# wenyuqing/panacea

Hardware: AMD Instinct MI355X
Metric: denoising steps/s (6-view x 8-frame 256x512) (higher is better)
Workload: dtype f16; 1 GPU; BASELINE config 3: Panacea+ stage-2 UNet+ControlNet, CFG 2 x 8 frames, 6 views, latent 32x384, hint 256x3072, Euler/LegacyDDPM 50-step schedule; precision=precise: split(stream,gn_stt,ff_out,stem,gn_head,gnt)+e4m3-lo, parallelism=single, graph=False, streams=2, hoisted_step_invariants=False, fused_step_tail=True

## Files before the change

panacea_amd/csrc/gemm_dispatch.h:

```cpp
#pragma once
#include "gemm_kernel.h"

namespace pnc_gemm {

template <unsigned EPI, bool WS>
static int launch_ln(const PncGemmParams& p, hipStream_t st, TileChoice tc, const void* wlo16) {
    if (tc.tile == T_256x320) return launch<PNC_A_PLAIN, 256, 320, 4, 2, 2, false, EPI, WS>(p, st, 1, wlo16);
    return launch<PNC_A_PLAIN, 128, 128, 2, 2, 2, true, EPI, WS>(p, st, 1, wlo16);
}

template <bool WS>
int dispatch_plain(const PncGemmParams& p, unsigned epi, hipStream_t st, bool* ln_fused, const void* wlo16) {
    constexpr int AM = PNC_A_PLAIN;
    const TileChoice tc = choose_tile(p);
    if (epi & E_LN) {
        if (ln_whole_rows(p, tc)) *ln_fused = true;
        else epi &= ~E_LN;
    }
    if (tc.tile == T_128x32 && epi != E_O16 && epi != E_O32) epi = E_GENERIC;
    if constexpr (!WS) {
        if (tc.tile == T_256x320 && tc.ksplit == 1 && plain_persist_ok(p, epi)) {
            switch (epi) {
                case E_O16: return launch_plain_persist<E_O16>(p, st);
                case E_O16 | E_VT: return launch_plain_persist<E_O16 | E_VT>(p, st);
// ... 15 lines not shown
    switch (epi) {
        case E_O16: return launch_tile<AM, E_O16, WS>(p, st, tc, wlo16);
        case E_O16 | E_VT: return launch_tile<AM, E_O16 | E_VT, WS>(p, st, tc, wlo16);
        case E_O32: return launch_tile<AM, E_O32, WS>(p, st, tc, wlo16);
        case E_O32 | E_O16: return launch_tile<AM, E_O32 | E_O16, WS>(p, st, tc, wlo16);
        case E_R1 | E_O32: return launch_tile<AM, E_R1 | E_O32, WS>(p, st, tc, wlo16);
        case E_R1 | E_O32 | E_O16: return launch_tile<AM, E_R1 | E_O32 | E_O16, WS>(p, st, tc, wlo16);
        case E_R1 | E_O16: return launch_tile<AM, E_R1 | E_O16, WS>(p, st, tc, wlo16);
        case E_RB | E_O32: return launch_tile<AM, E_RB | E_O32, WS>(p, st, tc, wlo16);
        case E_O32 | E_LN: return launch_ln<E_O32 | E_LN, WS>(p, st, tc, wlo16);
        case E_RB | E_O32 | E_LN: return launch_ln<E_RB | E_O32 | E_LN, WS>(p, st, tc, wlo16);
        case E_R1 | E_O32 | E_LN: return launch_ln<E_R1 | E_O32 | E_LN, WS>(p, st, tc, wlo16);
        case E_GEGLU | E_O16:
            if (tc.tile == T_256x256 && geglu_persist_ok(p)) return launch_geglu_persist<256, 256, 4, 2, WS>(p, st, wlo16);
            return launch_tile<AM, E_GEGLU | E_O16, WS>(p, st, tc, wlo16);
        case E_O16 | E_GELU:
            if constexpr (!WS) {
                if (tc.tile == T_256x256) return launch<AM, 256, 256, 4, 2, 2, true, E_O16 | E_GELU>(p, st);
                return launch<AM, 128, 128, 2, 2, 2, true, E_O16 | E_GELU>(p, st);
            }
            break;
        default: break;
    }
    return launch_tile<AM, E_GENERIC, WS>(p, st, tc, wlo16);
}

template <bool WS>
int dispatch_conv3x3(const PncGemmParams& p, unsigned epi, hipStream_t st, const void* wlo16) {
    constexpr int AM = PNC_A_CONV3X3;
    if (const int geometry = conv3x3_tile_geometry(p, epi)) return dispatch_conv3x3_tiles<WS>(p, epi, geometry, st, wlo16);
    const TileChoice tc = choose_tile(p);
    if (tc.tile == T_128x32 && epi != E_O16 && epi != E_O32) epi = E_GENERIC;
    switch (epi) {
        case E_O16: return launch_tile<AM, E_O16, WS>(p, st, tc, wlo16);
        case E_O32: return launch_tile<AM, E_O32, WS>(p, st, tc, wlo16);
        case E_O32 | E_O16: return launch_tile<AM, E_O32 | E_O16, WS>(p, st, tc, wlo16);
        case E_R1 | E_O32: return launch_tile<AM, E_R1 | E_O32, WS>(p, st, tc, wlo16);
        case E_R1 | E_O32 | E_O16: return launch_tile<AM, E_R1 | E_O32 | E_O16, WS>(p, st, tc, wlo16);
        default: return launch_tile<AM, E_GENERIC, WS>(p, st, tc, wlo16);
    }
}

static inline bool gn_stats_in_epilogue(const PncGemmParams& p, const TileChoice& tc) {
    const int cpg = p.N / 32;
    return tc.tile == T_256x320 && (p.N % 320) == 0 && (160 % cpg) == 0 && (cpg % 2) == 0 && (p.Npix % 64) == 0 && (p.M % 64) == 0 &&
           pnc_get_option(PNC_OPT_GEMM_GN_STATS) != 0;
}

template <bool WS>
int dispatch_conv1d(const PncGemmParams& p, unsigned epi, hipStream_t st, const void* wlo16) {
    constexpr int AM = PNC_A_CONV1D_T;
    TileChoice tc = choose_tile(p);
    if (tc.tile == T_128x32) epi = E_GENERIC;
    if (p.gn_part) {
        if (gn_stats_in_epilogue(p, tc)) {
            switch (epi) {
                case E_R1 | E_RB | E_O32: return launch<AM, 256, 320, 4, 2, 2, false, E_R1 | E_RB | E_O32 | E_GS, WS>(p, st, 1, wlo16);
                case E_R1 | E_R2 | E_O32: return launch<AM, 256, 320, 4, 2, 2, false, E_R1 | E_R2 | E_O32 | E_GS, WS>(p, st, 1, wlo16);
                case E_R1 | E_R2 | E_O32 | E_O16: return launch<AM, 256, 320, 4, 2, 2, false, E_R1 | E_R2 | E_O32 | E_O16 | E_GS, WS>(p, st, 1, wlo16);
                default: break;
            }
        }
        PncGemmParams q = p;
        q.gn_part = nullptr;
        const int rc = dispatch_conv1d<WS>(q, epi, st, wlo16);
        if (rc != PNC_OK) return rc;
        return pnc_groupnorm_stats(p.out32, p.ldc32, p.M / p.Npix, p.Npix, p.N, 64, p.gn_part, st);
    }
    switch (epi) {
        case E_R1 | E_RB | E_O32: return launch_tile<AM, E_R1 | E_RB | E_O32, WS>(p, st, tc, wlo16);
        case E_R1 | E_R2 | E_O32: return launch_tile<AM, E_R1 | E_R2 | E_O32, WS>(p, st, tc, wlo16);
        case E_R1 | E_R2 | E_O32 | E_O16: return launch_tile<AM, E_R1 | E_R2 | E_O32 | E_O16, WS>(p, st, tc, wlo16);
        default: return launch_tile<AM, E_GENERIC, WS>(p, st, tc, wlo16);
    }
}

}
```

panacea_amd/csrc/gemm_glds_body.inc:

```
    PncGemmParams p = pin;
    constexpr int NW = WGM * WGN;
    constexpr int MI = BM / WGM / 32, NI = BN / WGN / 32;
    constexpr int RPI = NW * 8;
    constexpr int A_IT = BM / RPI, B_IT = BN / RPI;
    constexpr int LOADS = A_IT + B_IT;
    constexpr int A_BYTES = BM * 128, B_BYTES = BN * 128, STAGE = A_BYTES + B_BYTES;
    static_assert(BM % RPI == 0 && BN % RPI == 0, "tile rows must be a multiple of the DMA row group");
    constexpr int ENI = NI < 2 ? NI : 2;
    constexpr int EPITCH = ENI * 32 + 4;
    constexpr bool GEGLU = (EPI & E_GEGLU) != 0;
    extern __shared__ __attribute__((aligned(16))) char smem[];

    const half_t* __restrict__ A = reinterpret_cast<const half_t*>(p.A);
    const half_t* __restrict__ A_lo = reinterpret_cast<const half_t*>(p.A_lo);
    const half_t* __restrict__ Wt = reinterpret_cast<const half_t*>(p.W);

    const int tiles_n = (p.N + BN - 1) / BN;
    const int tiles_m = (p.M + BM - 1) / BM;
    const int ntile_mn = tiles_m * tiles_n;
    int kslice = 0, tile, part = 0;
    if (ksplit > 1) {
        const int blk = xcd_remap(blockIdx.x, ntile_mn * ksplit);
        kslice = blk / ntile_mn; tile = blk - kslice * ntile_mn;
    } else if ((int)blockIdx.x < nfull) {
// ... 388 lines not shown
            for (int kt = 0; kt < nt_w; ++kt) {
                const bool ahead = (kt + 2) < ntot;
                if (ahead) issue_tile(kt + 2, st == 0 ? 2 : st - 1);
                if (wave_on) {
                    compute(st);
                    if (kt + 1 == nt_w) scale_lo();
                }
                if (ahead) asm volatile("s_waitcnt vmcnt(%0)" ::"n"(LOADS) : "memory");
                else asm volatile("s_waitcnt vmcnt(0)" ::: "memory");
                asm volatile("s_waitcnt lgkmcnt(0)" ::: "memory");
                __builtin_amdgcn_s_barrier();
                st = (st == 2) ? 0 : st + 1;
            }
        }
        for (int kt = nt_w; kt < n8; ++kt) {
            const bool ahead = (kt + 2) < ntot;
            if (ahead) issue_tile(kt + 2, st == 0 ? 2 : st - 1);
            if (wave_on) compute8(st, kt - nt_w);
            if (ahead) asm volatile("s_waitcnt vmcnt(%0)" ::"n"(LOADS) : "memory");
            else asm volatile("s_waitcnt vmcnt(0)" ::: "memory");
            asm volatile("s_waitcnt lgkmcnt(0)" ::: "memory");
            __builtin_amdgcn_s_barrier();
            st = (st == 2) ? 0 : st + 1;
        }
        for (int kt = n8; kt < ntot; ++kt) {
            const bool ahead = (kt + 2) < ntot;
            if (ahead) issue_tile(kt + 2, st == 0 ? 2 : st - 1);
            if (wave_on) {
                compute(st);
                if (!WS && !lo8 && kt + 1 == nt_lo) scale_lo();
            }
            if (ahead) asm volatile("s_waitcnt vmcnt(%0)" ::"n"(LOADS) : "memory");
            else asm volatile("s_waitcnt vmcnt(0)" ::: "memory");
            asm volatile("s_waitcnt lgkmcnt(0)" ::: "memory");
            __builtin_amdgcn_s_barrier();
            st = (st == 2) ? 0 : st + 1;
        }
    }

    if (!wave_on) return;
    const int mw = m0 + wm * (MI * 32), nw = n0 + wn * (NI * 32);
    if constexpr ((EPI & E_GENERIC) != 0) {
        epi_generic<MI, NI>(p, acc, lane, mw, nw);
    } else {
        if constexpr ((EPI & E_VT) != 0) {
            if (n0 >= p.n_split) { epi_vt<MI, NI>(p, acc, lane, mw, nw); return; }
        }
        if constexpr (EPI == (E_R1 | E_O32) || EPI == E_O32) {
            if (direct_epi && p.act == PNC_ACT_NONE && m0 + BM <= p.M && n0 + BN <= p.N && !split_rows && ksplit == 1) {
                epi_direct_o32<MI, NI, (EPI & E_R1) != 0>(p, acc, lane, RowLinear{mw}, nw);
                return;
            }
        }
        float* ep = reinterpret_cast<float*>(smem) + wave * (32 * EPITCH);
        __syncthreads();
        if constexpr (GEGLU) {
            epi_geglu<MI, NI>(p, acc, ep, lane, mw, nw, reinterpret_cast<const float*>(smem + RING_BYTES));
        } else {
            if constexpr ((EPI & E_LN) != 0) {
                static_assert(WGN == 2, "the fused LayerNorm pairs the two waves of a row");
                float2* lnb = reinterpret_cast<float2*>(reinterpret_cast<float*>(smem) + NW * (32 * EPITCH));
                epi_fast<MI, NI, EPI>(p, acc, ep, lane, RowLinear{mw}, nw, p.N, lnb + wave * 64, lnb + (wave ^ 1) * 64);
            } else {
                float* gs_tab = reinterpret_cast<float*>(smem) + NW * (32 * EPITCH) + wave * (NI * 16);
                epi_fast<MI, NI, (EPI & ~E_VT)>(p, acc, ep, lane, RowLinear{mw}, nw, (EPI & E_VT) ? p.n_split : p.N, nullptr, nullptr,
                                                (EPI & E_GS) ? gs_tab : nullptr);
            }
        }
    }
```

panacea_amd/csrc/gemm_kernel.h:

```cpp
#pragma once
#include "common.h"
#include <atomic>
#include <utility>

namespace pnc_gemm {

constexpr int BK = 64;
constexpr int BK8 = 128;
typedef int i32x4 __attribute__((ext_vector_type(4)));
typedef int i32x8 __attribute__((ext_vector_type(8)));
constexpr int E8M0_LO_INV = 127 - 11;

enum : unsigned {
    E_R1 = 1,
    E_R2 = 2,
    E_RB = 4,
    E_O32 = 8,
    E_O16 = 16,
    E_VT = 32,
    E_GEGLU = 64,
    E_GENERIC = 128,
    E_GELU = 256,
    E_LN = 512,
    E_GS = 1024
// ... 94 lines not shown
        int tap, ci;
        if ((p.Cin & 63) == 0) {
            const int cc = kc / 192, r = kc - cc * 192;
            tap = r >> 6; ci = (cc << 6) + (r & 63);
        } else {
            tap = kc / p.Cin; ci = kc - tap * p.Cin;
        }
        const int tt = s.y + tap - 1;
        return (!p.t_halo && (tt < 0 || tt >= p.T)) ? PNC_BUF_OOB : (unsigned)(s.rel + (tap - 1) * p.Npix * p.Cin + ci) * ESZ;
    }
}

__device__ __forceinline__ f32x4 ld4(const float* p) { return *reinterpret_cast<const f32x4*>(p); }

__device__ __forceinline__ float gelu_erf_f(float v) { return 0.5f * v * (1.0f + erff(v * 0.70710678118654752440f)); }
__device__ __attribute__((noinline)) static float gelu_erf_call(float v) { return gelu_erf_f(v); }

__device__ __forceinline__ void store_h8(half_t* out16, void* out16_lo, int64_t off, const float (&v)[8], int lo_fmt = PNC_LO_F16) {
    half8v o;
#pragma unroll
    for (int e = 0; e < 8; ++e) o[e] = (half_t)v[e];
    *reinterpret_cast<half8v*>(out16 + off) = o;
    if (out16_lo) {
        float r[8];
#pragma unroll
        for (int e = 0; e < 8; ++e) r[e] = (v[e] - (float)o[e]) * LO_SCALE;
        if (lo_fmt == PNC_LO_E4M3) {
            uint2 w;
            w.x = pack4_e4m3(r[0], r[1], r[2], r[3]);
            w.y = pack4_e4m3(r[4], r[5], r[6], r[7]);
            *reinterpret_cast<uint2*>(reinterpret_cast<char*>(out16_lo) + off) = w;
        } else {
            half8v l;
#pragma unroll
            for (int e = 0; e < 8; ++e) l[e] = (half_t)r[e];
            *reinterpret_cast<half8v*>(reinterpret_cast<half_t*>(out16_lo) + off) = l;
        }
    }
}

struct RowLinear {
    int mw;
    __device__ __forceinline__ int operator()(int lr) const { return mw + lr; }
};
template <int TWS>
struct RowHalo {
    int base, W, lr0;
    __device__ __forceinline__ int operator()(int lr) const {
        const int R = lr0 + lr;
        return base + (R >> TWS) * W + (R & ((1 << TWS) - 1));
    }
};

template <int MI, int NI, unsigned EPI, class RM = RowLinear>
__device__ __forceinline__ void epi_fast(const PncGemmParams& p, f32x16 (&acc)[MI][NI], float* ep, int lane,
                                         RM rmap, int nw, int ncols, float2* ln_mine = nullptr,
                                         const float2* ln_partner = nullptr, float* gs_tab = nullptr) {
    constexpr bool R1 = (EPI & E_R1) != 0, R2 = (EPI & E_R2) != 0, RB = (EPI & E_RB) != 0;
    constexpr bool O32 = (EPI & E_O32) != 0, O16 = (EPI & E_O16) != 0, LN = (EPI & E_LN) != 0;
    constexpr bool GS = (EPI & E_GS) != 0;
    static_assert(!GS || (O32 && !LN), "statistics of the fp32 output; not next to the fused LayerNorm");
    const int cpg = GS ? (p.N >> 5) : 1;
    if constexpr (GS) {
        gs_tab[lane] = 0.0f;
        if (lane + 64 < NI * 16) gs_tab[lane + 64] = 0.0f;
    }
    static_assert(!LN || O32, "the fused LayerNorm normalises the fp32 output it has just written");
    constexpr bool HAS_X = R1 || RB, HAS_Y = R1 && (R2 || RB);
    static_assert(!(R2 && !R1), "a single residual is passed as res1");
    static_assert(!(R1 && R2 && RB), "three added streams run the generic epilogue");
    constexpr int ENI = NI < 2 ? NI : 2;
    constexpr int EPITCH = ENI * 32 + 4;
    constexpr int NJ = (NI + ENI - 1) / ENI, NS = NJ * MI;
    constexpr int NPMAX = ENI == 2 ? 4 : 2;
    half_t* out16 = reinterpret_cast<half_t*>(p.out16);
    void* out16_lo = p.out16_lo;
    constexpr bool GELU = (EPI & E_GELU) != 0;
    const bool silu = (!HAS_X) && (p.act == PNC_ACT_SILU);
    const f32x4 z4 = {0.0f, 0.0f, 0.0f, 0.0f};
    f32x4 x0[NPMAX], x1[NPMAX], y0[NPMAX], y1[NPMAX];
    if constexpr (LN) {
        if (lane < MI * 32) ln_mine[lane] = make_float2(0.0f, 0.0f);
    }

    auto load_xy = [&](auto s_, auto ps_) {
        constexpr int s = decltype(s_)::value, ps = decltype(ps_)::value;
        constexpr int jc = (s / MI) * ENI, i = s % MI, cw = (NI - jc) < ENI ? (NI - jc) : ENI;
        constexpr int CPL = cw * 4, RPP = 64 / CPL;
        const int cl = lane % CPL, rl = lane / CPL;
        const int ncol = nw + jc * 32 + cl * 8;
        const int m = rmap(i * 32 + ps * RPP + rl);
        const bool on = (m < p.M) && (ncol < ncols);
        if constexpr (HAS_X) {
            x0[ps] = z4; x1[ps] = z4;
            if (on) {
                const float* xp = R1 ? p.res1 + (int64_t)m * p.ldr1 + ncol
                                     : p.rowbias + (int64_t)((m / p.rb_rows) % p.rb_mod) * p.N + ncol;
                x0[ps] = ld4(xp); x1[ps] = ld4(xp + 4);
            }
        }
        if constexpr (HAS_Y) {
            y0[ps] = z4; y1[ps] = z4;
            if (on) {
                const float* yp = R2 ? p.res2 + (int64_t)m * p.ldr2 + ncol
                                     : p.rowbias + (int64_t)((m / p.rb_rows) % p.rb_mod) * p.N + ncol;
                y0[ps] = ld4(yp); y1[ps] = ld4(yp + 4);
// ... 77 lines not shown
                float* dst = ep + (ps * RPP + rl) * EPITCH + cl * 8;
                *reinterpret_cast<f32x4*>(dst) = f32x4{v[0], v[1], v[2], v[3]};
                *reinterpret_cast<f32x4*>(dst + 4) = f32x4{v[4], v[5], v[6], v[7]};
            }
            if constexpr (GS) {
                if (on) {
#pragma unroll
                    for (int k = 0; k < 4; ++k) {
                        gP[k] += v[2 * k] + v[2 * k + 1];
                        gQ[k] += fmaf(v[2 * k], v[2 * k], v[2 * k + 1] * v[2 * k + 1]);
                    }
                }
            }
            if (!on) return;
            if constexpr (O32) {
                float* op = p.out32 + (int64_t)m * p.ldc32 + ncol;
                const f32x4 o0 = {v[0], v[1], v[2], v[3]}, o1 = {v[4], v[5], v[6], v[7]};
                *reinterpret_cast<f32x4*>(op) = o0;
                *reinterpret_cast<f32x4*>(op + 4) = o1;
            }
            if constexpr (O16) store_h8(out16, out16_lo, (int64_t)m * p.ldc16 + ncol, v, p.out_lo_fmt);
        });
        if constexpr (GS) {
            const int nA = min(8, (ncol / cpg + 1) * cpg - ncol);
            float sA = 0.0f, qA = 0.0f, sB = 0.0f, qB = 0.0f;
#pragma unroll
            for (int k = 0; k < 4; ++k) {
                const bool a = 2 * k < nA;
                sA += a ? gP[k] : 0.0f; qA += a ? gQ[k] : 0.0f;
                sB += a ? 0.0f : gP[k]; qB += a ? 0.0f : gQ[k];
            }
#pragma unroll
            for (int o = CPL; o < 64; o <<= 1) {
                sA += __shfl_xor(sA, o, 64); qA += __shfl_xor(qA, o, 64);
                sB += __shfl_xor(sB, o, 64); qB += __shfl_xor(qB, o, 64);
            }
            if (lane < CPL) {
                f32x4* e = reinterpret_cast<f32x4*>(gs_tab + (jc * 4 + cl) * 4);
                f32x4 t = *e;
                t[0] += sA; t[1] += qA; t[2] += sB; t[3] += qB;
                *e = t;
            }
        }
        if constexpr (LN) {
            asm volatile("s_waitcnt lgkmcnt(0)" ::: "memory");
            static_for<cw>([&](auto j_) {
                constexpr int j = decltype(j_)::value;
#pragma unroll
                for (int r = 0; r < 16; ++r)
                    acc[i][jc + j][r] = ep[mfma32_row(r, lane) * EPITCH + j * 32 + (lane & 31)];
            });
        }
    });
    if constexpr (GS) {
        asm volatile("s_waitcnt lgkmcnt(0)" ::: "memory");
        const int m_first = rmap(0);
        if (lane < (NI * 32) / cpg && m_first < p.M) {
            const int c0 = (lane * cpg) >> 3, c1 = ((lane + 1) * cpg - 1) >> 3;
            float S = 0.0f, Q = 0.0f;
            for (int c = c0; c <= c1; ++c) {
                const f32x4 t = *reinterpret_cast<const f32x4*>(gs_tab + c * 4);
                const bool first = (c * 8) / cpg == lane;
                S += first ? t[0] : t[2];
                Q += first ? t[1] : t[3];
            }
            const float n = (float)(MI * 32 * cpg);
            const float mean = S / n;
            const int f = m_first / p.Npix, chunk = (m_first - f * p.Npix) / (MI * 32), nrec = p.Npix / (MI * 32);
            float* o = p.gn_part + ((int64_t)(f * nrec + chunk) * 32 + nw / cpg + lane) * 3;
            o[0] = n; o[1] = mean; o[2] = fmaxf(Q - S * mean, 0.0f);
        }
    }
    if constexpr (LN) {
        __syncthreads();
        half_t* lnout = reinterpret_cast<half_t*>(p.ln_out16);
        const float invn = 1.0f / (float)p.N;
        static_for<NS>([&](auto s_) {
            constexpr int s = decltype(s_)::value, jc = (s / MI) * ENI, i = s % MI;
            constexpr int cw = (NI - jc) < ENI ? (NI - jc) : ENI;
            constexpr int CPL = cw * 4, RPP = 64 / CPL, NP = 32 / RPP;
            const int cl = lane % CPL, rl = lane / CPL;
            const int ncol = nw + jc * 32 + cl * 8;
            const bool col_on = ncol < ncols;
            f32x4 g0 = z4, g1 = z4, h0 = z4, h1 = z4;
            if (col_on) {
                g0 = ld4(p.ln_gamma + ncol); g1 = ld4(p.ln_gamma + ncol + 4);
                h0 = ld4(p.ln_beta + ncol); h1 = ld4(p.ln_beta + ncol + 4);
            }
            asm volatile("s_waitcnt lgkmcnt(0)" ::: "memory");
            static_for<cw>([&](auto j_) {
                constexpr int j = decltype(j_)::value;
#pragma unroll
                for (int r = 0; r < 16; ++r)
                    ep[mfma32_row(r, lane) * EPITCH + j * 32 + (lane & 31)] = acc[i][jc + j][r];
            });
            asm volatile("s_waitcnt lgkmcnt(0)" ::: "memory");
            f32x4 w0[NP], w1[NP];
#pragma unroll
            for (int ps = 0; ps < NP; ++ps) {
                const float* src = ep + (ps * RPP + rl) * EPITCH + cl * 8;
                w0[ps] = ld4(src); w1[ps] = ld4(src + 4);
            }
#pragma unroll
            for (int ps = 0; ps < NP; ++ps) {
                const int r = i * 32 + ps * RPP + rl;
                const int m = rmap(r);
                if (!(col_on && m < p.M)) continue;
                const float2 a = ln_mine[r], b = ln_partner[r];
                const float mean = (a.x + b.x) * invn;
                const float var = fmaxf(fmaf(-mean, mean, (a.y + b.y) * invn), 0.0f);
                const float rs = rsqrtf(var + p.ln_eps);
                float y[8];
#pragma unroll
                for (int e = 0; e < 4; ++e) {
                    y[e] = fmaf((w0[ps][e] - mean) * rs, g0[e], h0[e]);
                    y[e + 4] = fmaf((w1[ps][e] - mean) * rs, g1[e], h1[e]);
                }
                store_h8(lnout, nullptr, (int64_t)m * p.ldln + ncol, y);
            }
        });
    }
}

template <int MI, int NI>
__device__ __forceinline__ void epi_geglu(const PncGemmParams& p, f32x16 (&acc)[MI][NI], float* ep, int lane,
// ... 122 lines not shown
            snd.h = grp ? he : ho;
            rcv.w.x = __shfl_xor(snd.w.x, 32, 64);
            rcv.w.y = __shfl_xor(snd.w.y, 32, 64);
            half8v o8;
#pragma unroll
            for (int q = 0; q < 4; ++q) {
                o8[q] = grp ? rcv.h[q] : he[q];
                o8[4 + q] = grp ? ho[q] : rcv.h[q];
            }
            const int m8 = mw + i * 32 + 8 * (2 * rp + grp);
            if (col_on && m8 < p.M) {
                const int g = m8 / p.t_rows, t0 = m8 - g * p.t_rows;
                *reinterpret_cast<half8v*>(out16t + (int64_t)g * p.t_gstride + (int64_t)(n - p.n_split) * p.ldt + t0) = o8;
            }
        }
    });
}

template <int MI, int NI, bool R1, class RM>
__device__ __forceinline__ void epi_direct_o32(const PncGemmParams& p, f32x16 (&acc)[MI][NI], int lane, RM rmap, int nw) {
    const int col = lane & 31, h4 = 4 * (lane >> 5);
    const int m00 = rmap(0);
    const buffer_rsrc_t ro = make_rsrc(p.out32 + (int64_t)m00 * p.ldc32, 0x7FFFFF00u);
    const buffer_rsrc_t rr = make_rsrc(R1 ? p.res1 + (int64_t)m00 * p.ldr1 : p.out32, 0x7FFFFF00u);
    int vo[MI], vr[MI];
#pragma unroll
    for (int i = 0; i < MI; ++i) {
        const int dm = rmap(i * 32 + h4) - m00;
        vo[i] = (dm * p.ldc32 + nw + col) * 4;
        vr[i] = R1 ? (dm * p.ldr1 + nw + col) * 4 : 0;
    }
    unsigned x[2][16];
    auto load_res = [&](auto b_) {
        constexpr int b = decltype(b_)::value, i = b / NI, j = b % NI;
#pragma unroll
        for (int r = 0; r < 16; ++r) {
            const int so = (rmap((r & 3) + 8 * (r >> 2)) - m00) * p.ldr1 * 4;
            x[b & 1][r] = __builtin_amdgcn_raw_buffer_load_b32(rr, vr[i] + j * 128, so, 0);
        }
    };
    if constexpr (R1) load_res(std::integral_constant<int, 0>{});
    static_for<MI * NI>([&](auto b_) {
        constexpr int b = decltype(b_)::value, i = b / NI, j = b % NI;
        const float bn = p.bias ? p.bias[nw + j * 32 + col] : 0.0f;
        if constexpr (R1 && b + 1 < MI * NI) load_res(std::integral_constant<int, b + 1>{});
#pragma unroll
        for (int r = 0; r < 16; ++r) {
            float v = acc[i][j][r] + bn;
            if constexpr (R1) v += __builtin_bit_cast(float, x[b & 1][r]);
            const int so = (rmap((r & 3) + 8 * (r >> 2)) - m00) * p.ldc32 * 4;
            __builtin_amdgcn_raw_buffer_store_b32(__builtin_bit_cast(unsigned, v), ro, vo[i] + j * 128, so, 0);
        }
    });
}

template <int MI, int NI>
__device__ __forceinline__ void epi_generic(const PncGemmParams& p, f32x16 (&acc)[MI][NI], int lane, int mw, int nw) {
    half_t* out16 = reinterpret_cast<half_t*>(p.out16);
    half_t* out16_lo = reinterpret_cast<half_t*>(p.out16_lo);
    half_t* out16t = reinterpret_cast<half_t*>(p.out16t);
    const int col = lane & 31;
    static_for<MI * NI>([&](auto ij_) {
        constexpr int i = decltype(ij_)::value / NI, j = decltype(ij_)::value % NI;
        const int n = nw + j * 32 + col;
        if (n >= p.N) return;
        const float bn = p.bias ? p.bias[n] : 0.0f;
        const bool to_t = out16t && n >= p.n_split;
#pragma unroll 4
        for (int r = 0; r < 16; ++r) {
            const int m = mw + i * 32 + mfma32_row(r, lane);
            if (m >= p.M) continue;
            float v = acc[i][j][r] + bn;
            if (p.rowbias) v += p.rowbias[(int64_t)((m / p.rb_rows) % p.rb_mod) * p.N + n];
            if (p.act == PNC_ACT_SILU) v = silu_f(v);
            if (p.act == PNC_ACT_GELU) v = gelu_erf_call(v);
            if (p.res1) v += p.res1[(int64_t)m * p.ldr1 + n];
            if (p.res2) v += p.res2[(int64_t)m * p.ldr2 + n];
            if (to_t) {
                const int g = m / p.t_rows, t = m - g * p.t_rows;
                out16t[(int64_t)g * p.t_gstride + (int64_t)(n - p.n_split) * p.ldt + t] = (half_t)v;
                continue;
            }
            if (p.out32) p.out32[(int64_t)m * p.ldc32 + n] = v;
            if (out16) {
                const half_t h = (half_t)v;
                out16[(int64_t)m * p.ldc16 + n] = h;
                if (out16_lo) {
                    const float r = (v - (float)h) * LO_SCALE;
                    if (p.out_lo_fmt == PNC_LO_E4M3)
                        reinterpret_cast<unsigned char*>(p.out16_lo)[(int64_t)m * p.ldc16 + n] = (unsigned char)(pack4_e4m3(r, 0.0f, 0.0f, 0.0f) & 0xFFu);
                    else out16_lo[(int64_t)m * p.ldc16 + n] = (half_t)r;
                }
            }
        }
    });
}

template <int AMODE, int BM, int BN, int WGM, int WGN, int STAGES, bool PIPE, unsigned EPI>
__global__ __launch_bounds__(64 * WGM * WGN) void gemm_glds_kernel(const PncGemmParams pin, const int ksplit,
                                                                   const int nfull, const int tail_f,
                                                                   const float* __restrict__ phi_g, const int group_m,
                                                                   const int stagger_min_in) {
    constexpr bool WS = false;
    const void* const wlo16 = nullptr;
#include "gemm_glds_body.inc"
}
// ... 452 lines not shown
            if (nxt && !late) issue(m0, n0, kt + 1, (sp + kt + 1) & 1);
            compute((sp + kt) & 1, m0, n0, (nxt && late) ? kt + 1 : -1, (sp + kt + 1) & 1);
            __syncthreads();
        }
        const int vn = v + gridDim.x;
        int m1 = 0, n1 = 0;
        if (vn < ntile) {
            tile_origin(vn, m1, n1);
            issue(m1, n1, 0, 1);
        }
        if constexpr ((EPI & E_VT) != 0) {
            if (n0 >= p.n_split) epi_vt<MI, NI>(p, acc, lane, m0 + wm * (MI * 32), n0 + wn * (NI * 32));
            else epi_fast_alds<MI, NI, (EPI & ~E_VT)>(p, acc, ep, lane, m0 + wm * (MI * 32), n0 + wn * (NI * 32), 0u, 0u);
        } else if constexpr (EPI == E_O32 || EPI == (E_R1 | E_O32)) {
            if (!(group_m_in & 0x10000) && p.act == PNC_ACT_NONE)
                epi_direct_o32<MI, NI, (EPI & E_R1) != 0>(p, acc, lane, RowLinear{m0 + wm * (MI * 32)}, n0 + wn * (NI * 32));
            else
                epi_fast_alds<MI, NI, EPI>(p, acc, ep, lane, m0 + wm * (MI * 32), n0 + wn * (NI * 32), lnb + (unsigned)wave * 512u,
                                           lnb + (unsigned)(wave ^ 1) * 512u);
        } else {
            epi_fast_alds<MI, NI, EPI>(p, acc, ep, lane, m0 + wm * (MI * 32), n0 + wn * (NI * 32), lnb + (unsigned)wave * 512u,
                                       lnb + (unsigned)(wave ^ 1) * 512u);
        }
        if (vn >= ntile) break;
        alds_wait0();
        v = vn; m0 = m1; n0 = n1; sp = 1;
    }
}

static inline bool plain_persist_ok(const PncGemmParams& p, unsigned epi) {
    if ((pnc_get_option(PNC_OPT_GEMM_PERSIST) & 2) == 0 || p.a_mode != PNC_A_PLAIN) return false;
    if ((p.M % 256) || (p.N % 320) || (p.K % 64) || p.K < 64) return false;
    if (p.A_lo && (p.a_lo_fmt != PNC_LO_E4M3 || (p.lda % 16))) return false;
    if ((epi & E_LN) && p.N != 320) return false;
    if ((epi & E_VT) && ((p.n_split % 320) || (p.M % 8) || (p.t_rows % 8))) return false;
    return (p.M / 256) * (p.N / 320) >= 512;
}

template <unsigned EPI>
int launch_plain_persist(const PncGemmParams& p, hipStream_t st) {
    constexpr int lds = 2 * (256 + 320) * 128;
    static std::atomic<unsigned char> attr_done[64];
    const int dev = current_device();
    auto kern = gemm_persist_kernel<EPI>;
    set_dynamic_lds_once(attr_done, dev, kern, lds);
    const int tiles_n = p.N / 320, tiles_m = p.M / 256, tiles = tiles_m * tiles_n;
    const int group_m = grouped_tile_order(tiles_m, tiles_n);
    const int ncu = cu_count(dev);
    const int blocks = tiles < ncu ? tiles : ncu;
    hipLaunchKernelGGL(kern, dim3(blocks), dim3(512), lds, st, p, group_m | ((pnc_get_option(PNC_OPT_GEMM_FUSE_LN) & 2) ? 0x10000 : 0));
    return pnc_launch_status();
}

template <int AMODE, int BM, int BN, int WGM, int WGN, int STAGES, bool PIPE, unsigned EPI, bool WS = false>
int launch(const PncGemmParams& p, hipStream_t st, int ksplit = 1, const void* wlo16 = nullptr) {
    constexpr int lds = STAGES * (BM + BN) * 128;
    constexpr int threads = 64 * WGM * WGN;
    constexpr bool GEGLU = (EPI & E_GEGLU) != 0;
    static_assert(lds + (GEGLU ? PHI_BYTES : 0) <= 160 * 1024, "LDS budget of one CU (operand ring + GEGLU table)");
    static_assert(lds >= WGM * WGN * (32 * 68 * 4 + 64 * 8), "epilogue staging (+ LayerNorm row sums) must fit the operand ring");
    static std::atomic<unsigned char> attr_done[64];
    const auto kern = [] {
        if constexpr (WS) return gemm_glds_ws_kernel<AMODE, BM, BN, WGM, WGN, STAGES, PIPE, EPI>;
        else return gemm_glds_kernel<AMODE, BM, BN, WGM, WGN, STAGES, PIPE, EPI>;
    }();
    set_dynamic_lds_once(attr_done, current_device(), kern, lds + (GEGLU ? PHI_BYTES : 0));
    const int tiles =((p.M + BM - 1) / BM) * ((p.N + BN - 1) / BN);
    int nfull = tiles, tail_f = 1;
    if (ksplit == 1) tail_split<BM, WGM, lds>(tiles, nfull, tail_f);
    const int blocks = ksplit > 1 ? tiles * ksplit : nfull + (tiles - nfull) * tail_f;
    PncGemmParams q = p;
    const float* phi = nullptr;
    if constexpr (GEGLU) {
        int rc = PNC_OK;
        phi = phi_table_device(st, &rc);
        if (rc != PNC_OK) return rc;
    }
    if (ksplit > 1) {
        q.ldc32 = p.N;
        q.bias = nullptr; q.rowbias = nullptr; q.res1 = nullptr; q.res2 = nullptr;
        q.out16 = nullptr; q.out16_lo = nullptr; q.out16t = nullptr; q.n_split = p.N; q.act = PNC_ACT_NONE;
    }
    const int group_m = grouped_tile_order((p.M + BM - 1) / BM, (p.N + BN - 1) / BN);
    const int stagger = (pnc_get_option(PNC_OPT_GEMM_STAGGER) & 0xFF) | ((pnc_get_option(PNC_OPT_GEMM_FUSE_LN) & 2) ? 0 : 0x100);
    launch_kernel<WS>(kern, dim3(blocks), dim3(threads), lds + (GEGLU ? PHI_BYTES : 0), st, wlo16, q, ksplit, nfull, tail_f, phi, group_m, stagger);
    if (ksplit > 1) return launch_splitk_reduce(p, ksplit, st);
    return pnc_launch_status();
}

static inline double tile_score(long tiles, int slots, double eff) {
    if (tiles <= 0) return 0.0;
    const long q = tiles / slots, r = tiles % slots;
    const double tail = r == 0 ? 0.0 : (r * 4 <= slots ? 0.45 : (r * 2 <= slots ? 0.65 : 1.0));
    return eff * ((double)tiles / slots) / ((double)q + tail);
}

static inline int splitk_slices(const PncGemmParams& p) {
    if (p.geglu || p.out16t || (p.N % 256) || (p.N % 8)) return 1;
    if ((p.out32 && (p.ldc32 % 4)) || (p.out16 && (p.ldc16 % 8))) return 1;
    const long tiles = (long)((p.M + 255) / 256) * (p.N / 256);
    const int ktiles = (p.K + BK - 1) / BK;
    if (tiles > 96 || ktiles < 48) return 1;
    return ktiles >= 320 ? 8 : (ktiles >= 56 ? 4 : 2);
}

enum { T_128x128 = 1, T_256x128 = 2, T_256x320 = 3, T_256x256 = 4, T_128x32 = 5 };
// ... 52 lines not shown
```

panacea_amd/csrc/misc.hip:

```cpp
#include "common.h"
#include <atomic>

namespace {

constexpr int SM_MAXM = 16;

__global__ __launch_bounds__(256) void linear_smallm_kernel(const float* __restrict__ a, int lda,
                                                            const half_t* __restrict__ W,
                                                            const half_t* __restrict__ W_lo,
                                                            const float* __restrict__ bias,
                                                            float* __restrict__ out, int ldo, int M, int N,
                                                            int K, int silu_in, int silu_out) {
    const int lane = threadIdx.x & 63;
    const int n = blockIdx.x * 4 + (threadIdx.x >> 6);
    if (n >= N) return;
    float acc[SM_MAXM];
#pragma unroll
    for (int m = 0; m < SM_MAXM; ++m) acc[m] = 0.0f;
    for (int k0 = lane * 8; k0 < K; k0 += 64 * 8) {
        const half8v w = *reinterpret_cast<const half8v*>(W + (int64_t)n * K + k0);
        float wf[8];
#pragma unroll
        for (int e = 0; e < 8; ++e) wf[e] = (float)w[e];
        if (W_lo) {
// ... 329 lines not shown
    case PNC_SAMPLER_LMS:
        nv = 2 + p.n_hist;
        ok = p.out_aux && p.n_hist >= 0 && p.n_hist <= 3;
        for (int k = 0; ok && k < p.n_hist; ++k) ok = p.hist[k] != nullptr;
        break;
    default: return PNC_EINVAL;
    }
    for (int k = 0; ok && k < nv; ++k) ok = p.v[k] != nullptr;
    if (!ok) return PNC_EINVAL;
    return launch_1d(skip ? cfg_sampler_step_kernel<true> : cfg_sampler_step_kernel<false>, (int64_t)p.T * p.Npix, stream, p,
                     c_skip);
}

int cfg_euler_step_launch(const float* eps_tok, int ld, int T, int Npix, int C, int cfg, float scale, const float* x,
                          const float* c_out, const float* sigma, const float* sigma_next, float* x_next, const float* c_skip,
                          bool skip, void* stream) {
    PncSamplerStepParams p = {};
    p.struct_bytes = (int32_t)sizeof(PncSamplerStepParams);
    p.mode = PNC_SAMPLER_HEUN1;
    p.eps_tok = eps_tok, p.ld = ld, p.T = T, p.Npix = Npix, p.C = C, p.cfg = cfg, p.scale = scale;
    p.x = x, p.c_out = c_out, p.v[0] = sigma, p.v[1] = sigma_next, p.out = x_next;
    return cfg_sampler_step_launch(&p, c_skip, skip, true, stream);
}

}

extern "C" int pnc_cfg_euler_step(const float* eps_tok, int ld, int T, int Npix, int C, int cfg, float scale,
                                  const float* x, const float* c_out, const float* sigma, const float* sigma_next,
                                  float* x_next, void* stream) {
    return cfg_euler_step_launch(eps_tok, ld, T, Npix, C, cfg, scale, x, c_out, sigma, sigma_next, x_next, nullptr, false, stream);
}

extern "C" int pnc_cfg_euler_step_skip(const float* eps_tok, int ld, int T, int Npix, int C, int cfg, float scale,
                                       const float* x, const float* c_skip, const float* c_out, const float* sigma,
                                       const float* sigma_next, float* x_next, void* stream) {
    return cfg_euler_step_launch(eps_tok, ld, T, Npix, C, cfg, scale, x, c_out, sigma, sigma_next, x_next, c_skip, true, stream);
}

extern "C" int pnc_cfg_sampler_step(const PncSamplerStepParams* pp, void* stream) {
    return cfg_sampler_step_launch(pp, nullptr, false, false, stream);
}

extern "C" int pnc_cfg_sampler_step_skip(const PncSamplerStepParams* pp, const float* c_skip, void* stream) {
    return cfg_sampler_step_launch(pp, c_skip, true, false, stream);
}

extern "C" const char* pnc_version(void) { return "panacea_hip 0.4.0 gfx950"; }
#ifndef PNC_BUILD_DIGEST
#define PNC_BUILD_DIGEST "unstamped"
#endif
static const char k_build_digest[] = "pnc-build-digest:" PNC_BUILD_DIGEST;
extern "C" const char* pnc_build_digest(void) { return k_build_digest + 17; }

static std::atomic<int> g_options[PNC_OPT_COUNT] = {{1}, {0}, {0}, {1}, {1}, {0}, {1}, {3}, {8}, {1}, {4}, {12}};

int pnc_get_option(int option) { return g_options[option].load(std::memory_order_relaxed); }

extern "C" int pnc_set_option(int option, int value) {
    if (option < 0 || option >= PNC_OPT_COUNT) return PNC_EINVAL;
    return g_options[option].exchange(value, std::memory_order_relaxed);
}

extern "C" int pnc_linear_smallm_split(const float* a, int lda, const void* W, const void* W_lo, const float* bias,
                                       float* out, int ldo, int M, int N, int K, int silu_in, int silu_out,
                                       void* stream) {
    if (!a || !W || !out || M < 1 || M > SM_MAXM || N < 1 || K < 8) return PNC_EINVAL;
    if (K % 8 || lda % 4) return PNC_EINVAL;
    if (((uintptr_t)a | (uintptr_t)W | (uintptr_t)W_lo) & 15) return PNC_EALIGN;
    return launch_1d(linear_smallm_kernel, (int64_t)N * 64, stream, a, lda, f16p(W), f16p(W_lo), bias, out, ldo, M, N, K, silu_in,
                     silu_out);
}

extern "C" int pnc_linear_smallm(const float* a, int lda, const void* W, const float* bias,
                                 float* out, int ldo, int M, int N, int K, int silu_in, int silu_out,
                                 void* stream) {
    return pnc_linear_smallm_split(a, lda, W, nullptr, bias, out, ldo, M, N, K, silu_in, silu_out, stream);
}

extern "C" int pnc_linear_smallm_segments(const float* a, int lda, const void* W, const float* bias, float* out, int M,
                                          int m0, int Mtot, int N, int K, const int32_t* seg_start, int nseg, int silu_in,
                                          int silu_out, void* stream) {
    return pnc_linear_smallm_segments_split(a, lda, W, nullptr, bias, out, M, m0, Mtot, N, K, seg_start, nseg, silu_in, silu_out, stream);
}

extern "C" int pnc_linear_smallm_segments_split(const float* a, int lda, const void* W, const void* W_lo, const float* bias,
                                                float* out, int M, int m0, int Mtot, int N, int K, const int32_t* seg_start,
                                                int nseg, int silu_in, int silu_out, void* stream) {
    if (!a || !W || !out || !seg_start || M < 1 || M > SM_MAXM || m0 < 0 || m0 + M > Mtot || N < 1 || K < 8) return PNC_EINVAL;
    if (K % 8 || lda % 4 || nseg < 1 || nseg > PNC_SMALLM_MAX_SEGS) return PNC_EINVAL;
    if (((uintptr_t)a | (uintptr_t)W | (uintptr_t)W_lo) & 15) return PNC_EALIGN;
    SmallmSegs segs;
    segs.nseg = nseg;
    if (seg_start[0] != 0 || seg_start[nseg] != N) return PNC_EINVAL;
    for (int i = 0; i <= nseg; ++i) {
        if (seg_start[i] % SEG_NC || (i > 0 && seg_start[i] <= seg_start[i - 1])) return PNC_EINVAL;
        segs.start[i] = seg_start[i];
    }
    return launch_1d(linear_smallm_seg_kernel, (int64_t)(N / SEG_NC) * 64, stream, a, lda, f16p(W), f16p(W_lo), bias, out, M, m0, Mtot,
                     N, K, silu_in, silu_out, segs);
}

template <typename TS>
static int timestep_embedding(const TS* t, int F, int dim, const float* freqs, float* out, void* stream) {
    if (!t || !out || !freqs || F < 1 || dim < 2) return PNC_EINVAL;
    return launch_1d(timestep_embedding_kernel<TS>, F * (dim / 2), stream, t, F, dim, freqs, out);
}

// ... 122 lines not shown
```

Measured before the change: 6.408 steps/s.

## Add persistent conv1d temporal GEMM kernel with direct residual and GN-stats epilogue

Adds a persistent conv1d (temporal) GEMM kernel for 256x320 tiles. It prefetches the next tile's first K-stage while the current tile's epilogue runs. It also adds a direct-to-global epilogue that fuses bias, row bias or second residual and GroupNorm partial statistics using DPP lane reductions, skipping the LDS staging round-trip. The default persist option is changed from 3 to 7 to enable the path, which adds code complexity and a new reduction ordering for GN statistics.

```diff
diff --git a/panacea_amd/csrc/gemm_dispatch.h b/panacea_amd/csrc/gemm_dispatch.h
--- a/panacea_amd/csrc/gemm_dispatch.h
+++ b/panacea_amd/csrc/gemm_dispatch.h
@@ -91,6 +91,17 @@
     constexpr int AM = PNC_A_CONV1D_T;
     TileChoice tc = choose_tile(p);
     if (tc.tile == T_128x32) epi = E_GENERIC;
+    if constexpr (!WS) {
+        if (tc.tile == T_256x320 && tc.ksplit == 1 && conv1d_persist_ok(p, epi) && (!p.gn_part || gn_stats_in_epilogue(p, tc))) {
+            switch (epi | (p.gn_part ? (unsigned)E_GS : 0u)) {
+                case E_R1 | E_RB | E_O32: return launch_conv1d_persist<E_R1 | E_RB | E_O32>(p, st);
+                case E_R1 | E_R2 | E_O32: return launch_conv1d_persist<E_R1 | E_R2 | E_O32>(p, st);
+                case E_R1 | E_RB | E_O32 | E_GS: return launch_conv1d_persist<E_R1 | E_RB | E_O32 | E_GS>(p, st);
+                case E_R1 | E_R2 | E_O32 | E_GS: return launch_conv1d_persist<E_R1 | E_R2 | E_O32 | E_GS>(p, st);
+                default: break;
+            }
+        }
+    }
     if (p.gn_part) {
         if (gn_stats_in_epilogue(p, tc)) {
             switch (epi) {
diff --git a/panacea_amd/csrc/gemm_glds_body.inc b/panacea_amd/csrc/gemm_glds_body.inc
--- a/panacea_amd/csrc/gemm_glds_body.inc
+++ b/panacea_amd/csrc/gemm_glds_body.inc
@@ -464,6 +464,14 @@
                 return;
             }
         }
+        if constexpr (AMODE == PNC_A_CONV1D_T && BM == 256 && BN == 320 &&
+                      ((EPI & ~E_GS) == (E_R1 | E_RB | E_O32) || (EPI & ~E_GS) == (E_R1 | E_R2 | E_O32))) {
+            if (direct_epi && p.act == PNC_ACT_NONE && m0 + BM <= p.M && n0 + BN <= p.N && !split_rows && ksplit == 1 &&
+                (!(EPI & E_RB) || (p.rb_rows & 63) == 0)) {
+                epi_direct2_o32<MI, NI, EPI>(p, acc, lane, mw, nw);
+                return;
+            }
+        }
         float* ep = reinterpret_cast<float*>(smem) + wave * (32 * EPITCH);
         __syncthreads();
         if constexpr (GEGLU) {
diff --git a/panacea_amd/csrc/gemm_kernel.h b/panacea_amd/csrc/gemm_kernel.h
--- a/panacea_amd/csrc/gemm_kernel.h
+++ b/panacea_amd/csrc/gemm_kernel.h
@@ -170,6 +170,31 @@
     }
 };
 
+template <int MI>
+__device__ __forceinline__ void gs_store_record(const PncGemmParams& p, float S, float Q, int lane, int m_first, int nw, int cpg) {
+    const float n = (float)(MI * 32 * cpg);
+    const float mean = S / n;
+    const int f = m_first / p.Npix, chunk = (m_first - f * p.Npix) / (MI * 32), nrec = p.Npix / (MI * 32);
+    float* o = p.gn_part + ((int64_t)(f * nrec + chunk) * 32 + nw / cpg + lane) * 3;
+    o[0] = n; o[1] = mean; o[2] = fmaxf(Q - S * mean, 0.0f);
+}
+
+template <int MI, int NI>
+__device__ __forceinline__ void gs_write_records(const PncGemmParams& p, const float* gs_tab, int lane, int m_first, int nw, int cpg) {
+    asm volatile("s_waitcnt lgkmcnt(0)" ::: "memory");
+    if (lane < (NI * 32) / cpg && m_first < p.M) {
+        const int c0 = (lane * cpg) >> 3, c1 = ((lane + 1) * cpg - 1) >> 3;
+        float S = 0.0f, Q = 0.0f;
+        for (int c = c0; c <= c1; ++c) {
+            const f32x4 t = *reinterpret_cast<const f32x4*>(gs_tab + c * 4);
+            const bool first = (c * 8) / cpg == lane;
+            S += first ? t[0] : t[2];
+            Q += first ? t[1] : t[3];
+        }
+        gs_store_record<MI>(p, S, Q, lane, m_first, nw, cpg);
+    }
+}
+
 template <int MI, int NI, unsigned EPI, class RM = RowLinear>
 __device__ __forceinline__ void epi_fast(const PncGemmParams& p, f32x16 (&acc)[MI][NI], float* ep, int lane,
                                          RM rmap, int nw, int ncols, float2* ln_mine = nullptr,
@@ -353,25 +378,7 @@
             });
         }
     });
-    if constexpr (GS) {
-        asm volatile("s_waitcnt lgkmcnt(0)" ::: "memory");
-        const int m_first = rmap(0);
-        if (lane < (NI * 32) / cpg && m_first < p.M) {
-            const int c0 = (lane * cpg) >> 3, c1 = ((lane + 1) * cpg - 1) >> 3;
-            float S = 0.0f, Q = 0.0f;
-            for (int c = c0; c <= c1; ++c) {
-                const f32x4 t = *reinterpret_cast<const f32x4*>(gs_tab + c * 4);
-                const bool first = (c * 8) / cpg == lane;
-                S += first ? t[0] : t[2];
-                Q += first ? t[1] : t[3];
-            }
-            const float n = (float)(MI * 32 * cpg);
-            const float mean = S / n;
-            const int f = m_first / p.Npix, chunk = (m_first - f * p.Npix) / (MI * 32), nrec = p.Npix / (MI * 32);
-            float* o = p.gn_part + ((int64_t)(f * nrec + chunk) * 32 + nw / cpg + lane) * 3;
-            o[0] = n; o[1] = mean; o[2] = fmaxf(Q - S * mean, 0.0f);
-        }
-    }
+    if constexpr (GS) gs_write_records<MI, NI>(p, gs_tab, lane, rmap(0), nw, cpg);
     if constexpr (LN) {
         __syncthreads();
         half_t* lnout = reinterpret_cast<half_t*>(p.ln_out16);
@@ -600,6 +607,123 @@
             __builtin_amdgcn_raw_buffer_store_b32(__builtin_bit_cast(unsigned, v), ro, vo[i] + j * 128, so, 0);
         }
     });
+}
+
+__device__ __forceinline__ float dpp_xor1(float v) {
+    return __builtin_bit_cast(float, __builtin_amdgcn_update_dpp(0, __builtin_bit_cast(int, v), 0xB1, 0xF, 0xF, true));
+}
+__device__ __forceinline__ float dpp_shr2(float v) {
+    return __builtin_bit_cast(float, __builtin_amdgcn_update_dpp(0, __builtin_bit_cast(int, v), 0x112, 0xF, 0xF, true));
+}
+
+template <int MI, int NI, unsigned EPI>
+__device__ __forceinline__ void epi_direct2_o32(const PncGemmParams& p, f32x16 (&acc)[MI][NI], int lane, int mw, int nw) {
+    constexpr bool RB = (EPI & E_RB) != 0, R2 = (EPI & E_R2) != 0, GS = (EPI & E_GS) != 0;
+    static_assert((EPI & ~E_GS) == (E_R1 | E_RB | E_O32) || (EPI & ~E_GS) == (E_R1 | E_R2 | E_O32), "res1 + (row bias | res2), fp32 output");
+    constexpr int G = R2 ? 8 : 16, HB = 16 / G;
+    constexpr int NU = NI * MI * HB;
+    const int col = lane & 31, h4 = 4 * (lane >> 5);
+    const buffer_rsrc_t ro = make_rsrc(p.out32 + (int64_t)mw * p.ldc32, 0x7FFFFF00u);
+    const buffer_rsrc_t rx = make_rsrc(p.res1 + (int64_t)mw * p.ldr1, 0x7FFFFF00u);
+    const buffer_rsrc_t ry = make_rsrc(R2 ? p.res2 + (int64_t)mw * p.ldr2 : p.out32, 0x7FFFFF00u);
+    const float* rbp = RB ? p.rowbias + (int64_t)((mw / p.rb_rows) % p.rb_mod) * p.N + nw + col : nullptr;
+    int vo[MI], vx[MI], vy[MI];
+#pragma unroll
+    for (int i = 0; i < MI; ++i) {
+        const int dm = i * 32 + h4;
+        vo[i] = (dm * p.ldc32 + nw + col) * 4;
+        vx[i] = (dm * p.ldr1 + nw + col) * 4;
+        vy[i] = R2 ? (dm * p.ldr2 + nw + col) * 4 : 0;
+    }
+    unsigned x[2][G], y[R2 ? 2 : 1][R2 ? G : 1];
+    auto load_unit = [&](auto u_) {
+        constexpr int u = decltype(u_)::value, j = u / (MI * HB), i = (u / HB) % MI, hf = u % HB;
+#pragma unroll
+        for (int g = 0; g < G; ++g) {
+            const int r = hf * G + g, row = (r & 3) + 8 * (r >> 2);
+            x[u & 1][g] = __builtin_amdgcn_raw_buffer_load_b32(rx, vx[i] + j * 128, row * p.ldr1 * 4, 0);
+            if constexpr (R2) y[u & 1][g] = __builtin_amdgcn_raw_buffer_load_b32(ry, vy[i] + j * 128, row * p.ldr2 * 4, 0);
+        }
+    };
+    const int cpg = GS ? (p.N >> 5) : 1;
+    float gP[4][2], gQ[4][2], tab[4];
+    const int gc0 = (lane * cpg) >> 3, gc1 = ((lane + 1) * cpg - 1) >> 3;
+    float gS = 0.0f, gQs = 0.0f;
+    load_unit(std::integral_constant<int, 0>{});
+    static_for<NU>([&](auto u_) {
+        constexpr int u = decltype(u_)::value, j = u / (MI * HB), i = (u / HB) % MI, hf = u % HB;
+        constexpr bool odd = (NI & 1) != 0 && j == NI - 1;
+        const float bn = p.bias ? p.bias[nw + j * 32 + col] : 0.0f;
+        float rbv = 0.0f;
+        if constexpr (RB) rbv = rbp[j * 32];
+        if constexpr (u + 1 < NU) load_unit(std::integral_constant<int, u + 1>{});
+        if constexpr (GS && hf == 0) {
+#pragma unroll
+            for (int e = 0; e < 4; ++e) { gP[e][0] = gP[e][1] = 0.0f; gQ[e][0] = gQ[e][1] = 0.0f; }
+            if constexpr (i == 0) { tab[0] = tab[1] = tab[2] = tab[3] = 0.0f; }
+        }
+#pragma unroll
+        for (int g = 0; g < G; ++g) {
+            const int r = hf * G + g, row = (r & 3) + 8 * (r >> 2);
+            float v = acc[i][j][r] + bn;
+            if constexpr (RB) v += rbv;
+            v += __builtin_bit_cast(float, x[u & 1][g]);
+            if constexpr (R2) v += __builtin_bit_cast(float, y[u & 1][g]);
+            __builtin_amdgcn_raw_buffer_store_b32(__builtin_bit_cast(unsigned, v), ro, vo[i] + j * 128, row * p.ldc32 * 4, 0);
+            if constexpr (GS) {
+                const float w = dpp_xor1(v);
+                const int e = r & 3, ch = odd ? ((r >> 2) & 1) : 0;
+                gP[e][ch] += v + w;
+                gQ[e][ch] += fmaf(v, v, w * w);
+            }
+        }
+        if constexpr (GS && hf == HB - 1) {
+            const int ncol = nw + j * 32 + (col & ~7);
+            const int nA = min(8, (ncol / cpg + 1) * cpg - ncol);
+            const bool a = (col & 6) < nA;
+            constexpr int NCH = odd ? 2 : 1;
+            float fin[4][NCH];
+#pragma unroll
+            for (int ch = 0; ch < NCH; ++ch) {
+                float z[4][4];
+#pragma unroll
+                for (int e = 0; e < 4; ++e) {
+                    const float s[4] = {a ? gP[e][ch] : 0.0f, a ? gQ[e][ch] : 0.0f, a ? 0.0f : gP[e][ch], a ? 0.0f : gQ[e][ch]};
+#pragma unroll
+                    for (int t = 0; t < 4; ++t) {
+                        float X = 0.0f + s[t];
+#pragma unroll
+                        for (int k = 1; k < 4; ++k) X = dpp_shr2(X) + s[t];
+                        z[t][e] = X;
+                    }
+                }
+#pragma unroll
+                for (int t = 0; t < 4; ++t) {
+                    float W = (z[t][0] + z[t][1]) + (z[t][2] + z[t][3]);
+                    W += __shfl_xor(W, 32, 64);
+                    fin[t][ch] = W;
+                }
+            }
+#pragma unroll
+            for (int t = 0; t < 4; ++t) tab[t] += odd ? fin[t][0] + fin[t][NCH - 1] : fin[t][0];
+            if constexpr (i == MI - 1) {
+#pragma unroll
+                for (int cc = 0; cc < 4; ++cc) {
+                    const int c = j * 4 + cc;
+                    float t[4];
+#pragma unroll
+                    for (int q = 0; q < 4; ++q)
+                        t[q] = __builtin_bit_cast(float, __builtin_amdgcn_readlane(__builtin_bit_cast(int, tab[q]), cc * 8 + 6));
+                    const bool in = c >= gc0 && c <= gc1, first = (c * 8) / cpg == lane;
+                    gS = in ? gS + (first ? t[0] : t[2]) : gS;
+                    gQs = in ? gQs + (first ? t[1] : t[3]) : gQs;
+                }
+            }
+        }
+    });
+    if constexpr (GS) {
+        if (lane < (NI * 32) / cpg) gs_store_record<MI>(p, gS, gQs, lane, mw, nw, cpg);
+    }
 }
 
 template <int MI, int NI>
@@ -1158,6 +1282,187 @@
     return pnc_launch_status();
 }
 
+template <unsigned EPI>
+__global__ __launch_bounds__(512) void gemm_conv1d_persist_kernel(const PncGemmParams pin) {
+    PncGemmParams p = pin;
+    constexpr int AMODE = PNC_A_CONV1D_T;
+    constexpr int BM = 256, BN = 320, WGM = 4, WGN = 2;
+    constexpr int NW = WGM * WGN, MI = BM / WGM / 32, NI = BN / WGN / 32, RPI = NW * 8, A_IT = BM / RPI, B_IT = BN / RPI;
+    constexpr int A_BYTES = BM * 128, B_BYTES = BN * 128, STAGE = A_BYTES + B_BYTES;
+    extern __shared__ __attribute__((aligned(16))) char smem[];
+    const half_t* __restrict__ A = reinterpret_cast<const half_t*>(p.A);
+    const half_t* __restrict__ Wt = reinterpret_cast<const half_t*>(p.W);
+    const int tiles_n = p.N / BN, tiles_m = p.M / BM, ntile = tiles_m * tiles_n;
+    const bool lo8 = p.A_lo != nullptr;
+    const int ntiles = p.K / BK;
+    const int nt_lo = lo8 ? (p.K + BK8 - 1) / BK8 : 0;
+    const int ntot = ntiles + nt_lo;
+    const int tid = threadIdx.x, lane = tid & 63;
+    const int wave = __builtin_amdgcn_readfirstlane(tid >> 6);
+    const int wm = wave / WGN, wn = wave % WGN;
+    const int pb_n = p.Npix / BM, nbt = tiles_m / pb_n;
+    auto tile_origin = [&](int v, int& m0, int& n0) {
+        const int tile = xcd_remap(v, ntile);
+        const int tn = tile % tiles_n, tm = tile / tiles_n;
+        m0 = ((tm % nbt) * pb_n + tm / nbt) * BM; n0 = tn * BN;
+    };
+    f32x16 acc[MI][NI];
+    int v = blockIdx.x;
+    if (v >= ntile) return;
+    int m0, n0, sp = 0;
+    tile_origin(v, m0, n0);
+    bool first = true;
+    const bool late = wave >= 4 && ntot >= 8;
+    while (true) {
+        int lt = lane;
+        asm volatile("" : "+v"(lt));
+        const int srow = wave * 8 + (lt >> 3);
+        const int schunk = (lt & 7) ^ ((srow >> 1) & 7);
+        const int frow = lt & 31, fk = lt >> 5;
+        unsigned woff[B_IT];
+#pragma unroll
+        for (int i = 0; i < B_IT; ++i) woff[i] = (unsigned)((i * RPI + srow) * p.ldw + schunk * 8) * 2u;
+        auto issue = [&](int m0, int n0, int kt_local, int stage) {
+            char* sa = smem + stage * STAGE + wave * 1024;
+            char* sb = sa + A_BYTES;
+            const int m_win = max(0, m0 - p.Npix);
+            RowState row;
+            row.valid = true; row.x = 0; row.y = (m0 / p.Npix) % p.T; row.rel = (m0 - m_win + srow) * p.Cin;
+            const int64_t a_origin = (int64_t)m_win * p.Cin;
+            if (kt_local < nt_lo) {
+                int schunk8 = schunk, srow8 = srow;
+                asm volatile("" : "+v"(schunk8), "+v"(srow8));
+                const buffer_rsrc_t rs_alo = make_rsrc(reinterpret_cast<const char*>(p.A_lo) + a_origin, 0x7FFFFF00u);
+                const buffer_rsrc_t rs_wlo = make_rsrc(reinterpret_cast<const char*>(p.W_lo) + (int64_t)n0 * p.ldw_lo, 0x7FFFFF00u);
+                const int kc8 = kt_local * BK8 + schunk8 * 16;
+                const unsigned ks8 = (unsigned)kt_local * BK8;
+                const bool k_on = kc8 < p.K;
+                const unsigned a0 = a_chunk_off<AMODE, 1u>(p, row, kc8);
+#pragma unroll
+                for (int i = 0; i < A_IT; ++i)
+                    glds16_buf(rs_alo, a0 == PNC_BUF_OOB ? PNC_BUF_OOB : a0 + (unsigned)(i * RPI * p.Cin), 0u, sa + i * (RPI * 128));
+#pragma unroll
+                for (int i = 0; i < B_IT; ++i)
+                    glds16_buf(rs_wlo, k_on ? (unsigned)((i * RPI + srow8) * p.ldw_lo + schunk8 * 16) : PNC_BUF_OOB, ks8, sb + i * (RPI * 128));
+                return;
+            }
+            const buffer_rsrc_t rs_a = make_rsrc(A + a_origin, 0x7FFFFF00u);
+            const buffer_rsrc_t rs_w = make_rsrc(Wt + (int64_t)n0 * p.ldw, 0x7FFFFF00u);
+            const int kt = kt_local - nt_lo;
+            const unsigned a0 = a_chunk_off<AMODE>(p, row, kt * BK + schunk * 8);
+#pragma unroll
+            for (int i = 0; i < A_IT; ++i)
+                glds16_buf(rs_a, a0 == PNC_BUF_OOB ? PNC_BUF_OOB : a0 + (unsigned)(i * RPI * p.Cin) * 2u, 0u, sa + i * (RPI * 128));
+            const unsigned ks = (unsigned)kt * (BK * 2);
+#pragma unroll
+            for (int i = 0; i < B_IT; ++i) glds16_buf(rs_w, woff[i], ks, sb + i * (RPI * 128));
+        };
+        auto compute = [&](int stage, int mid_kt, int mid_stage) {
+            const char* sa = smem + stage * STAGE;
+            const char* sb = sa + A_BYTES;
+#pragma unroll
+            for (int ks = 0; ks < BK / 16; ++ks) {
+                half8v af[MI], bf[NI];
+#pragma unroll
+                for (int i = 0; i < MI; ++i)
+                    af[i] = *reinterpret_cast<const half8v*>(sa + lds_off128(wm * (MI * 32) + i * 32 + frow, ks * 2 + fk));
+#pragma unroll
+                for (int j = 0; j < NI; ++j)
+                    bf[j] = *reinterpret_cast<const half8v*>(sb + lds_off128(wn * (NI * 32) + j * 32 + frow, ks * 2 + fk));
+#pragma unroll
+                for (int i = 0; i < MI; ++i)
+#pragma unroll
+                    for (int j = 0; j < NI; ++j)
+                        acc[i][j] = __builtin_amdgcn_mfma_f32_32x32x16_f16(af[i], bf[j], acc[i][j], 0, 0, 0);
+                if (ks == 1 && mid_kt >= 0) issue(m0, n0, mid_kt, mid_stage);
+            }
+        };
+        auto compute8 = [&](int stage, int kt_local) {
+            const char* sa = smem + stage * STAGE;
+            const char* sb = sa + A_BYTES;
+            const int nwin = (p.K - kt_local * BK8) > 64 ? 2 : 1;
+#pragma unroll
+            for (int w = 0; w < 2; ++w) {
+                if (w < nwin) {
+                    i32x8 af[MI];
+#pragma unroll
+                    for (int i = 0; i < MI; ++i) {
+                        const int row = wm * (MI * 32) + i * 32 + frow;
+                        const i32x4 a0 = *reinterpret_cast<const i32x4*>(sa + lds_off128(row, w * 4 + fk * 2));
+                        const i32x4 a1 = *reinterpret_cast<const i32x4*>(sa + lds_off128(row, w * 4 + fk * 2 + 1));
+                        af[i] = __builtin_shufflevector(a0, a1, 0, 1, 2, 3, 4, 5, 6, 7);
+                    }
+#pragma unroll
+                    for (int j = 0; j < NI; ++j) {
+                        const int row = wn * (NI * 32) + j * 32 + frow;
+                        const i32x4 b0 = *reinterpret_cast<const i32x4*>(sb + lds_off128(row, w * 4 + fk * 2));
+                        const i32x4 b1 = *reinterpret_cast<const i32x4*>(sb + lds_off128(row, w * 4 + fk * 2 + 1));
+                        const i32x8 bf = __builtin_shufflevector(b0, b1, 0, 1, 2, 3, 4, 5, 6, 7);
+#pragma unroll
+                        for (int i = 0; i < MI; ++i)
+                            acc[i][j] = __builtin_amdgcn_mfma_scale_f32_32x32x64_f8f6f4(af[i], bf, acc[i][j], 0, 0, 0, E8M0_LO_INV, 0, p.w_lo_exp);
+                        __builtin_amdgcn_sched_barrier(0);
+                    }
+                }
+            }
+        };
+
+#pragma unroll
+        for (int i = 0; i < MI; ++i)
+#pragma unroll
+            for (int j = 0; j < NI; ++j)
+#pragma unroll
+                for (int r = 0; r < 16; ++r) acc[i][j][r] = 0.0f;
+        if (first) { issue(m0, n0, 0, 0); first = false; }
+        __syncthreads();
+        for (int kt = 0; kt < nt_lo; ++kt) {
+            if (kt + 1 < ntot) issue(m0, n0, kt + 1, (sp + kt + 1) & 1);
+            compute8((sp + kt) & 1, kt);
+            __syncthreads();
+        }
+        for (int kt = nt_lo; kt < ntot; ++kt) {
+            const bool nxt = kt + 1 < ntot;
+            if (nxt && !late) issue(m0, n0, kt + 1, (sp + kt + 1) & 1);
+            compute((sp + kt) & 1, (nxt && late) ? kt + 1 : -1, (sp + kt + 1) & 1);
+            __syncthreads();
+        }
+        const int vn = v + gridDim.x;
+        int m1 = 0, n1 = 0;
+        if (vn < ntile) {
+            tile_origin(vn, m1, n1);
+            issue(m1, n1, 0, 1);
+        }
+        epi_direct2_o32<MI, NI, EPI>(p, acc, lt, m0 + wm * (MI * 32), n0 + wn * (NI * 32));
+        if (vn >= ntile) break;
+        v = vn; m0 = m1; n0 = n1; sp = 1;
+    }
+}
+
+static inline bool conv1d_persist_ok(const PncGemmParams& p, unsigned epi) {
+    const int opt = pnc_get_option(PNC_OPT_GEMM_PERSIST);
+    if ((opt & 4) == 0 || (pnc_get_option(PNC_OPT_GEMM_FUSE_LN) & 2) != 0) return false;
+    if (p.a_mode != PNC_A_CONV1D_T || p.t_halo || p.act != PNC_ACT_NONE) return false;
+    if ((p.M % 256) || (p.N % 320) || (p.Cin % 64) || p.K != 3 * p.Cin) return false;
+    if (p.Npix < 256 || (p.Npix % 256) || p.T < 1 || (p.M % (p.T * p.Npix))) return false;
+    if (p.A_lo && p.a_lo_fmt != PNC_LO_E4M3) return false;
+    if ((epi & E_RB) && (p.rb_rows < 64 || (p.rb_rows % 64))) return false;
+    const int tiles = (p.M / 256) * (p.N / 320);
+    return (opt & 8) ? tiles > cu_count(current_device()) : tiles >= 512;
+}
+
+template <unsigned EPI>
+int launch_conv1d_persist(const PncGemmParams& p, hipStream_t st) {
+    constexpr int lds = 2 * (256 + 320) * 128;
+    static std::atomic<unsigned char> attr_done[64];
+    const int dev = current_device();
+    auto kern = gemm_conv1d_persist_kernel<EPI>;
+    set_dynamic_lds_once(attr_done, dev, kern, lds);
+    const int tiles = (p.M / 256) * (p.N / 320);
+    const int ncu = cu_count(dev);
+    hipLaunchKernelGGL(kern, dim3(tiles < ncu ? tiles : ncu), dim3(512), lds, st, p);
+    return pnc_launch_status();
+}
+
 template <int AMODE, int BM, int BN, int WGM, int WGN, int STAGES, bool PIPE, unsigned EPI, bool WS = false>
 int launch(const PncGemmParams& p, hipStream_t st, int ksplit = 1, const void* wlo16 = nullptr) {
     constexpr int lds = STAGES * (BM + BN) * 128;
diff --git a/panacea_amd/csrc/misc.hip b/panacea_amd/csrc/misc.hip
--- a/panacea_amd/csrc/misc.hip
+++ b/panacea_amd/csrc/misc.hip
@@ -405,7 +405,7 @@
 static const char k_build_digest[] = "pnc-build-digest:" PNC_BUILD_DIGEST;
 extern "C" const char* pnc_build_digest(void) { return k_build_digest + 17; }
 
-static std::atomic<int> g_options[PNC_OPT_COUNT] = {{1}, {0}, {0}, {1}, {1}, {0}, {1}, {3}, {8}, {1}, {4}, {12}};
+static std::atomic<int> g_options[PNC_OPT_COUNT] = {{1}, {0}, {0}, {1}, {1}, {0}, {1}, {7}, {8}, {1}, {4}, {12}};
 
 int pnc_get_option(int option) { return g_options[option].load(std::memory_order_relaxed); }
 
```

Result: no change. 6.402 steps/s (-0.1%).
